# openai/blocksparse

Hardware: AMD Instinct MI355X
Metric: bsmm_effective_tflops_4096x4096_bs32_d20 (higher is better)
Workload: dtype bf16

## Files before the change

### blocksparse_amd/csrc/bsmm_common.h

```cpp
#pragma once
#include <hip/hip_runtime.h>
#include <stdint.h>

namespace bsmm {

typedef float f32x16 __attribute__((ext_vector_type(16)));
typedef float f32x4 __attribute__((ext_vector_type(4)));
typedef __bf16 bf16x8 __attribute__((ext_vector_type(8)));
typedef _Float16 f16x8 __attribute__((ext_vector_type(8)));
typedef _Float16 f16x4 __attribute__((ext_vector_type(4)));
typedef short s16x4v __attribute__((ext_vector_type(4)));

struct DTf32 {
    typedef float T;
    static constexpr bool is16 = false;
    static __device__ __forceinline__ float to_f32(float v) { return v; }
    static __device__ __forceinline__ float from_f32(float v) { return v; }
};

struct DTf16 {
    typedef uint16_t T;
    static constexpr bool is16 = true;
    static __device__ __forceinline__ float to_f32(uint16_t v) { return (float)__builtin_bit_cast(_Float16, v); }
    static __device__ __forceinline__ uint16_t from_f32(float v) {
// ... 113 lines not shown
template <class DT>
__device__ __forceinline__ void mma32(const Frag32<DT, false>& a, const Frag32<DT, false>& b, f32x16& acc) {
#pragma unroll
    for (int t = 0; t < 16; ++t) acc = __builtin_amdgcn_mfma_f32_32x32x2f32(a.v[t], b.v[t], acc, 0, 0, 0);
}

template <class DT, bool IS16 = DT::is16>
struct Frag16;

template <class DT>
struct Frag16<DT, true> {
    static constexpr int KL = 8;
    static constexpr int KS = 32;
    uint4 q;
    __device__ __forceinline__ void zero() { q = zero_u4(); }
    __device__ __forceinline__ void load_contig(const uint16_t* p) { q = *reinterpret_cast<const uint4*>(p); }
    __device__ __forceinline__ void load_contig_lim(const uint16_t* p, int lim) { q = load8_u16_lim(p, lim); }
    __device__ __forceinline__ void load_strided(const uint16_t* p, size_t stride) { q = gather8_u16(p, stride); }
    __device__ __forceinline__ void load_strided_lim(const uint16_t* p, size_t stride, int lim) { q = gather8_u16_lim(p, stride, lim); }
};

template <class DT>
struct Frag16<DT, false> {
    static constexpr int KL = 4;
    static constexpr int KS = 16;
    float v[4];
    __device__ __forceinline__ void zero() { v[0] = v[1] = v[2] = v[3] = 0.f; }
    __device__ __forceinline__ void load_contig(const float* p) {
        float4 x = *reinterpret_cast<const float4*>(p);
        v[0] = x.x; v[1] = x.y; v[2] = x.z; v[3] = x.w;
    }
    __device__ __forceinline__ void load_contig_lim(const float* p, int lim) {
        if (lim >= 4) { load_contig(p); return; }
#pragma unroll
        for (int t = 0; t < 4; ++t) v[t] = (t < lim) ? p[t] : 0.f;
    }
    __device__ __forceinline__ void load_strided(const float* p, size_t stride) {
#pragma unroll
        for (int t = 0; t < 4; ++t) v[t] = p[(size_t)t * stride];
    }
    __device__ __forceinline__ void load_strided_lim(const float* p, size_t stride, int lim) {
#pragma unroll
        for (int t = 0; t < 4; ++t) v[t] = (t < lim) ? p[(size_t)t * stride] : 0.f;
    }
};

template <class DT>
__device__ __forceinline__ void mma16(const Frag16<DT, true>& a, const Frag16<DT, true>& b, f32x4& acc) {
    acc = DT::mfma16(a.q, b.q, acc);
}
template <class DT>
__device__ __forceinline__ void mma16(const Frag16<DT, false>& a, const Frag16<DT, false>& b, f32x4& acc) {
#pragma unroll
    for (int t = 0; t < 4; ++t) acc = __builtin_amdgcn_mfma_f32_16x16x4f32(a.v[t], b.v[t], acc, 0, 0, 0);
}

template <class DT>
__device__ __forceinline__ void atomic_accumulate(typename DT::T* p, float v) {
    if constexpr (!DT::is16) {
        __hip_atomic_fetch_add(p, v, __ATOMIC_RELAXED, __HIP_MEMORY_SCOPE_AGENT);
    } else {
        uintptr_t a = reinterpret_cast<uintptr_t>(p);
        uint32_t* wp = reinterpret_cast<uint32_t*>(a & ~(uintptr_t)3);
        const bool hi = (a & 2) != 0;
        uint32_t old = __hip_atomic_load(wp, __ATOMIC_RELAXED, __HIP_MEMORY_SCOPE_AGENT);
        uint32_t assumed;
        do {
            assumed = old;
            uint16_t cur = hi ? (uint16_t)(assumed >> 16) : (uint16_t)(assumed & 0xffffu);
            uint32_t nv = DT::from_f32(DT::to_f32(cur) + v);
            uint32_t nw = hi ? ((assumed & 0x0000ffffu) | (nv << 16)) : ((assumed & 0xffff0000u) | nv);
            old = atomicCAS(wp, assumed, nw);
        } while (old != assumed);
    }
}

typedef __bf16 bf16x2_t __attribute__((ext_vector_type(2)));
typedef float f32x2_t __attribute__((ext_vector_type(2)));
__device__ __forceinline__ uint32_t bf16_pack2(float lo, float hi) {
    const f32x2_t v = {lo, hi};
    return __builtin_bit_cast(uint32_t, __builtin_convertvector(v, bf16x2_t));
}

struct PtrList8 {
    const void* p[8];
};

__device__ __forceinline__ void glds16_asm(const void* gsrc, uint32_t lds_byte_addr) {
    unsigned keep;
    asm volatile("s_mov_b32 %0, m0\n\ts_mov_b32 m0, %2\n\ts_nop 0\n\tglobal_load_lds_dwordx4 %1, off\n\ts_mov_b32 m0, %0"
                 : "=&s"(keep)
                 : "v"(gsrc), "s"(lds_byte_addr)
                 : "memory");
}
__device__ __forceinline__ void glds16_asm_masked(const void* gsrc, uint32_t lds_byte_addr, uint64_t mask) {
    unsigned keep;
    asm volatile("s_mov_b32 %0, m0\n\ts_mov_b32 m0, %2\n\ts_mov_b64 exec, %3\n\ts_nop 0\n\tglobal_load_lds_dwordx4 %1, off\n\t"
                 "s_mov_b64 exec, -1\n\ts_mov_b32 m0, %0"
                 : "=&s"(keep)
                 : "v"(gsrc), "s"(lds_byte_addr), "s"(mask)
                 : "memory");
}
__device__ __forceinline__ uint32_t lds_addr_of(const void* p) {
    return (uint32_t)(uintptr_t)(__attribute__((address_space(3))) const void*)p;
}

}
```

### blocksparse_amd/csrc/bsmm_updat_v2.h

```cpp
#pragma once
#include <type_traits>

#include "bsmm_common.h"
#include "bsmm_plan.h"
#include "bsmm_updat_tr.h"

namespace bsmm {

#ifndef U2_NT_PARTS
#define U2_NT_PARTS 1
#endif
#ifndef U2_MAX_SLICES
#define U2_MAX_SLICES 8
#endif
#ifndef U2_CH_ROWS
#define U2_CH_ROWS 16
#endif
#ifndef U2_SETB_FROM
#define U2_SETB_FROM 0
#endif
constexpr int U2_CH = U2_CH_ROWS;
constexpr int U2_KS = U2_CH / 16;
constexpr int U2_D = 64 / U2_CH;
constexpr int U2_AHEAD = U2_D / 2;
static_assert(U2_CH == 16 || U2_CH == 32, "chunk = 1 or 2 K-steps");
constexpr int u2_ring(int ws) { return ws == 32 ? 2 : U2_D; }
constexpr int u2_lds_bytes(int ws) { return u2_ring(ws) * 2 * U2_CH * ws * 64; }
constexpr int U2_CH0 = 32;
#ifndef U2_RING5
#define U2_RING5 0
#endif
constexpr int u2_lds_bytes0(int ws) { return U2_RING5 ? 5 * ws * 32 * (U2_CH0 * 2) : 131072; }

#ifdef U2_STAMPS
__device__ unsigned long long g_u2_trace[1024 * 8];
#define U2_STAMP(k, v) do { if (wave == 0 && lane == 0 && blockIdx.x < 1024) g_u2_trace[blockIdx.x * 8 + (k)] = (v); } while (0)
#else
#define U2_STAMP(k, v) do { } while (0)
#endif

__device__ __forceinline__ const void* uniform_ptr(const void* p) {
    const uint64_t v = reinterpret_cast<uint64_t>(p);
    const uint32_t lo = __builtin_amdgcn_readfirstlane((uint32_t)v), hi = __builtin_amdgcn_readfirstlane((uint32_t)(v >> 32));
    return reinterpret_cast<const void*>(((uint64_t)hi << 32) | lo);
}

__device__ __forceinline__ void glds16_saddr(const void* sbase, uint32_t voff, uint32_t lds_byte_addr) {
    unsigned keep;
    asm volatile("s_mov_b32 %0, m0\n\ts_mov_b32 m0, %3\n\ts_nop 0\n\tglobal_load_lds_dwordx4 %1, %2\n\ts_mov_b32 m0, %0"
                 : "=&s"(keep)
                 : "v"(voff), "s"(sbase), "s"(lds_byte_addr)
                 : "memory");
}
__device__ __forceinline__ void glds16_saddr_x2(const void* sbase, uint32_t voff0, uint32_t voff1, uint32_t lds_byte_addr) {
    unsigned keep;
    asm volatile("s_mov_b32 %0, m0\n\ts_mov_b32 m0, %4\n\ts_nop 0\n\tglobal_load_lds_dwordx4 %1, %3\n\t"
                 "s_add_u32 m0, m0, 0x400\n\ts_nop 0\n\tglobal_load_lds_dwordx4 %2, %3\n\ts_mov_b32 m0, %0"
                 : "=&s"(keep)
                 : "v"(voff0), "v"(voff1), "s"(sbase), "s"(lds_byte_addr)
                 : "memory", "scc");
}

__device__ __forceinline__ void glds16_saddr_x4(const void* sbase, uint32_t v0, uint32_t v1, uint32_t v2, uint32_t v3, uint32_t lds_byte_addr) {
    unsigned keep;
    asm volatile("s_mov_b32 %0, m0\n\ts_mov_b32 m0, %6\n\ts_nop 0\n\tglobal_load_lds_dwordx4 %1, %5\n\t"
                 "s_add_u32 m0, m0, 0x400\n\ts_nop 0\n\tglobal_load_lds_dwordx4 %2, %5\n\t"
                 "s_add_u32 m0, m0, 0x400\n\ts_nop 0\n\tglobal_load_lds_dwordx4 %3, %5\n\t"
                 "s_add_u32 m0, m0, 0x400\n\ts_nop 0\n\tglobal_load_lds_dwordx4 %4, %5\n\ts_mov_b32 m0, %0"
                 : "=&s"(keep)
                 : "v"(v0), "v"(v1), "v"(v2), "v"(v3), "s"(sbase), "s"(lds_byte_addr)
                 : "memory", "scc");
}

__device__ __forceinline__ const unsigned char* pick_ptr(const PtrList8& l, int idx) {
    const void* p = l.p[0];
#pragma unroll
    for (int k = 1; k < 8; ++k) p = (idx == k) ? l.p[k] : p;
    return static_cast<const unsigned char*>(p);
}

template <class DT, int LDSB>
__device__ __forceinline__ void u2_direct_block(const PtrList8& Xs, const PtrList8& Es, float* __restrict__ scratch, const int32_t* __restrict__ plan,
                                                int N, int Cf, int Kf, int pcount, int e, long region0, unsigned char* smem) {
    typedef typename DT::T T;
    constexpr int SLOT = 2048, D = LDSB / U2_WAVES / SLOT;
    static_assert(D >= 2 && LDSB >= U2_WAVES * 4096, "direct blocks: a ring of two chunks per wave and 64 KiB for the reduction");
    const int lane = threadIdx.x & 63;
    const int wave = __builtin_amdgcn_readfirstlane(threadIdx.x >> 6);
    const int DP = plan[30];
    const int d = e / DP, q = e - d * DP;
    const int32_t* de = plan + plan[29] + 4 * d;
    const int c = __builtin_amdgcn_readfirstlane(de[1]), k = __builtin_amdgcn_readfirstlane(de[2]);
    unsigned char* ring = smem + wave * (D * SLOT);
    const uint32_t ring_addr = lds_addr_of(ring);
    const int drow = lane >> 2, dpiece = lane & 3;
    const int g16 = lane >> 4, t16 = lane & 15, h = g16 >> 1;
    const int rd_base = (8 * h + (t16 >> 2)) * 64 + (16 * (g16 & 1) + 4 * (t16 & 3)) * 2;
    f32x16 acc;
#pragma unroll
    for (int i = 0; i < 16; ++i) acc[i] = 0.f;
    const int nch = (N + 15) >> 4;
    const int lo = (int)((long)nch * q / DP), hi = (int)((long)nch * (q + 1) / DP);
    const int first = lo + wave;
    const int myq = hi > first ? (hi - first + U2_WAVES - 1) / U2_WAVES : 0;
    for (int p = 0; p < pcount; ++p) {
        const T* X = reinterpret_cast<const T*>(pick_ptr(Xs, p)) + c * 32 + dpiece * 8;
        const T* E = reinterpret_cast<const T*>(pick_ptr(Es, p)) + k * 32 + dpiece * 8;
        auto issue = [&](int j, int pos) {
            const int r = min((first + U2_WAVES * j) * 16 + drow, N - 1);
            const uint32_t slot = __builtin_amdgcn_readfirstlane(ring_addr + pos * SLOT);
            glds16_asm(X + (size_t)r * Cf, slot);
            glds16_asm(E + (size_t)r * Kf, slot + 1024);
        };
#pragma unroll
        for (int j = 0; j < D - 1; ++j) issue(j, j);
        int rd_pos = 0, wr_pos = D - 1;
        for (int j = 0; j < myq; ++j) {
            issue(j + D - 1, wr_pos);
            asm volatile("s_waitcnt vmcnt(%0)" ::"n"(2 * (D - 1)) : "memory");
            const unsigned char* sp = ring + rd_pos * SLOT + rd_base;
            rd_pos = (rd_pos + 1 == D) ? 0 : rd_pos + 1;
            wr_pos = (wr_pos + 1 == D) ? 0 : wr_pos + 1;
            const uint2 a0 = ds_tr16(sp), a1 = ds_tr16(sp + 4 * 64), b0 = ds_tr16(sp + 1024), b1 = ds_tr16(sp + 1024 + 4 * 64);
            uint4 a = make_uint4(a0.x, a0.y, a1.x, a1.y);
            const uint4 b = make_uint4(b0.x, b0.y, b1.x, b1.y);
            const int nb = (first + U2_WAVES * j) * 16 + 8 * h;
            if (nb + 8 > N) {
                uint32_t* u = reinterpret_cast<uint32_t*>(&a);
#pragma unroll
                for (int i = 0; i < 4; ++i) u[i] &= ((nb + 2 * i < N) ? 0xffffu : 0u) | ((nb + 2 * i + 1 < N) ? 0xffff0000u : 0u);
            }
            asm volatile("s_waitcnt lgkmcnt(0)" ::: "memory");
            acc = DT::mfma32(a, b, acc);
        }
        asm volatile("s_waitcnt vmcnt(0)" ::: "memory");
    }
    __syncthreads();
    float* red = reinterpret_cast<float*>(smem);
#pragma unroll
    for (int reg = 0; reg < 16; ++reg) red[wave * 1024 + reg * 64 + lane] = acc[reg];
    __syncthreads();
    float sum = 0.f;
#pragma unroll
    for (int v = 0; v < U2_WAVES; ++v) sum += red[v * 1024 + threadIdx.x];
    const int reg = threadIdx.x >> 6, ln = threadIdx.x & 63;
    float* region = scratch + ((size_t)region0 * (U2_WAVES * U2_SLOTS) + (size_t)e) * 1024;
    region[((reg >> 2) * 64 + ln) * 4 + (reg & 3)] = sum;
}

template <class DT, int WS, int AXIS = 1>
__global__ void __launch_bounds__(64 * U2_WAVES, 4)
updat32_a1_v2_kernel(PtrList8 Xs, PtrList8 Es, typename DT::T* __restrict__ DW, float* __restrict__ scratch,
                     const int32_t* __restrict__ plan, int N, int Cf, int Kf, int pcount, float alpha, float beta, int flat, int main_grid, int rounds) {
    typedef typename DT::T T;
    static_assert(DT::is16 && (WS == 8 || WS == 16 || (WS == 32 && AXIS == 1)), "updat v2: 16-bit storage types, 8x8 / 16x16 windows (32x32: feature axis 1)");
    extern __shared__ __attribute__((aligned(16))) unsigned char smem[];
    constexpr int CH = AXIS == 1 ? U2_CH : U2_CH0;
    constexpr int KS = CH / 16;
    constexpr bool FIVE = AXIS == 0 && U2_RING5;
    constexpr int D = AXIS == 1 ? u2_ring(WS) : (WS == 16 ? 2 : 4);
    constexpr int AHEAD = D / 2;
    constexpr int ROWB = AXIS == 1 ? WS * 64 : CH * 2;
    constexpr int SLAB = AXIS == 1 ? CH * ROWB : WS * 32 * ROWB;
    constexpr int SLOT = 2 * SLAB;
    constexpr int PPR = ROWB / 16;
    constexpr int RPI = ROWB <= 1024 ? 1024 / ROWB : 1;
    constexpr int IPR = ROWB <= 1024 ? 1 : ROWB / 1024;
    constexpr int IPO = SLAB / 1024;
    constexpr int NI = 2 * IPO / U2_WAVES;
    static_assert((NI == 1 || NI == 2 || NI == 4) && NI * U2_WAVES == 2 * IPO && IPO % NI == 0, "the chunk must split evenly over the waves");

    const int mg = main_grid > 0 ? main_grid : (int)gridDim.x;
    if ((int)blockIdx.x >= mg) {
        if constexpr (AXIS == 1) u2_direct_block<DT, u2_lds_bytes(WS)>(Xs, Es, scratch, plan, N, Cf, Kf, pcount, (int)blockIdx.x - mg, (long)rounds * mg, smem);
        return;
    }
    const int lane = threadIdx.x & 63;
    const int wave = __builtin_amdgcn_readfirstlane(threadIdx.x >> 6);
    const int32_t* items = plan + plan[6];
    const int nchunks = (N + CH - 1) / CH;
    const int nfull = N / CH;
    const int CPI = pcount * nchunks;
    const bool xcd_mode = flat == 0 && (mg & 7) == 0;
    const int nsets = xcd_mode ? plan[8] : 1;
    const int nparts = xcd_mode ? 8 / nsets : 1;
    const int U = xcd_mode ? mg >> 3 : mg;
    const int xcd = xcd_mode ? (blockIdx.x & 7) : 0, uj = xcd_mode ? (blockIdx.x >> 3) : blockIdx.x;
    const int set = xcd / nparts, part = xcd - set * nparts;
    const int set_first = xcd_mode ? plan[9 + 2 * set] : 0, set_count = xcd_mode ? plan[10 + 2 * set] : plan[4];
    const int part_lo = (int)((long)part * CPI / nparts), part_hi = (int)((long)(part + 1) * CPI / nparts);
    const int full_rounds = set_count / U, m_last = set_count - full_rounds * U;
    const int k_last = m_last > 0 ? min(U / m_last, U2_MAX_SLICES) : 0;
    const int total_rounds = full_rounds + ((m_last > 0 && uj < m_last * k_last) ? 1 : 0);

    const uint32_t base_addr = lds_addr_of(smem);
    const int opE = (NI * wave) / IPO;
    const int ii0 = (NI * wave) % IPO;
    const int d_row0 = ROWB <= 1024 ? ii0 * RPI + lane / PPR : ii0 / IPR;
    auto row_of = [&](int q) -> int { return ROWB <= 1024 ? d_row0 + q * RPI : (ii0 + q) / IPR; };
    auto pos_of = [&](int q) -> int { return ROWB <= 1024 ? lane % PPR : ((ii0 + q) % IPR) * 64 + lane; };
    const uint32_t sub_off = ii0 * 1024;
    const uint32_t wave_off = (!FIVE ? opE * SLAB : 0) + sub_off;
    constexpr uint32_t HS = SLAB, RING0 = 5 * SLAB;
    const int F = opE ? Kf : Cf;
    const int my_piece0 = (lane % PPR) ^ ((d_row0 >> 2) & 3);
    const int g16 = lane >> 4, t16 = lane & 15;
    const int h = AXIS == 1 ? g16 >> 1 : lane >> 5;
    const int trow = t16 >> 2;
    const int tsub = (2 * (g16 & 1) + ((t16 & 3) >> 1)) * 16 + (t16 & 1) * 8;
    const int frag_row = AXIS == 1 ? (8 * h + trow) * ROWB + tsub : (lane & 31) * ROWB + ((h ^ (((lane & 31) >> 2) & 3)) << 4);
#ifdef U2_NO_PINGPONG
    const bool setb = false;
#else
    constexpr int SB = U2_SETB_FROM > 0 ? U2_SETB_FROM : ((WS == 8 && AXIS == 1) ? 4 : U2_WAVES / 2);
    const bool setb = wave >= SB;
#endif

    U2_STAMP(0, __builtin_amdgcn_s_memrealtime());
    U2_STAMP(4, (unsigned long long)total_rounds);
    for (int round = 0; round < total_rounds; ++round) {
        int item, r0, cnt;
        if (round < full_rounds) {
            item = set_first + round * U + uj;
            r0 = part_lo; cnt = part_hi - part_lo;
        } else {
            const int which = uj / k_last, slice = uj - which * k_last, L = part_hi - part_lo;
            item = set_first + full_rounds * U + which;
            r0 = part_lo + (int)((long)slice * L / k_last);
            cnt = part_lo + (int)((long)(slice + 1) * L / k_last) - r0;
        }
// ... 176 lines not shown
                    else     asm volatile("s_waitcnt vmcnt(%0)" ::"n"(NI) : "memory");
                }
                if (nfull != nchunks) {
                    if (cq == nfull) {
#pragma unroll
                        for (int e = 0; e < NI; ++e)
                            if (AXIS == 1 ? (cq * CH + row_of(e) >= N) : (cq * CH + my_piece0 * 8 >= N))
                                *reinterpret_cast<uint4*>(smem + (!FIVE ? (uint32_t)(i & (D - 1)) * SLOT : (uint32_t)((2 * i + opE) % 5) * HS) + wave_off + e * 1024 + lane * 16) = zero_u4();
                        asm volatile("s_waitcnt lgkmcnt(0)" ::: "memory");
                    }
                    if (++cq == nchunks) cq = 0;
                }
                if constexpr ((D == 2 || FIVE) && SETB) asm volatile("s_waitcnt lgkmcnt(0)" ::: "memory");
#ifndef U2_NO_BARRIER
                __builtin_amdgcn_s_barrier();
#endif
                const unsigned char* slot = smem + (!FIVE ? vslot : vslot0);
                const unsigned char* slot_y = smem + vslot;
                if constexpr (N0 == 0) {
                    U2_ISSUE();
                } else if constexpr (!SETB) {
                    read_frags(slot, slot_y, 0);
                    U2_ISSUE();
                    multiply();
#pragma unroll
                    for (int ks = 1; ks < KS; ++ks) { read_frags(slot, slot_y, ks); multiply(); }
                } else {
                    multiply();
                    __builtin_amdgcn_sched_barrier(0);
                    U2_ISSUE();
#pragma unroll
                    for (int ks = 0; ks < KS - 1; ++ks) { read_frags(slot, slot_y, ks); multiply(); }
                    read_frags(slot, slot_y, KS - 1);
                }
                if constexpr (!FIVE) {
                    vslot = (vslot + SLOT) & (D * SLOT - 1);
                } else {
                    vslot += 2 * HS;  vslot = vslot >= RING0 ? vslot - RING0 : vslot;
                    vslot0 += 2 * HS; vslot0 = vslot0 >= RING0 ? vslot0 - RING0 : vslot0;
                }
            }
#undef U2_ISSUE
#undef U2_ISSUE_SLOW
#undef U2_DMA1
#undef U2_DMA2
#undef U2_DMA4
            if constexpr (SETB && N0 > 0) multiply();
            asm volatile("s_waitcnt vmcnt(0)" ::: "memory");
            __builtin_amdgcn_s_barrier();
        };
        using std::integral_constant;
#define RUN(A, B)                                                                                                          \
    do {                                                                                                                   \
        if (setb) run(integral_constant<int, A>{}, integral_constant<int, B>{}, integral_constant<bool, true>{});          \
        else      run(integral_constant<int, A>{}, integral_constant<int, B>{}, integral_constant<bool, false>{});         \
    } while (0)
        switch (n0 * 8 + n1) {
            case 0 * 8 + 0: RUN(0, 0); break;
            case 1 * 8 + 0: RUN(1, 0); break;
            case 1 * 8 + 1: RUN(1, 1); break;
            case 1 * 8 + 2: RUN(1, 2); break;
            case 1 * 8 + 3: RUN(1, 3); break;
            case 2 * 8 + 0: RUN(2, 0); break;
            case 2 * 8 + 1: RUN(2, 1); break;
            case 2 * 8 + 2: RUN(2, 2); break;
            case 3 * 8 + 0: RUN(3, 0); break;
            case 3 * 8 + 1: RUN(3, 1); break;
            default:        RUN(4, 0); break;
        }
#undef RUN
        if (round == 0) { U2_STAMP(1, __builtin_amdgcn_s_memrealtime()); U2_STAMP(5, (unsigned long long)cnt); }

        if (scratch != nullptr) {
            float4* reg_base = reinterpret_cast<float4*>(scratch) + ((size_t)(round * mg + blockIdx.x) * (U2_WAVES * U2_SLOTS) + wave * U2_SLOTS) * 256 + lane;
#pragma unroll
            for (int j = 0; j < U2_SLOTS; ++j) {
                if (j >= n0 + n1) break;
#ifdef U2_NO_EPILOGUE
                if (alpha != 12345.f) continue;
#endif
#pragma unroll
                for (int q = 0; q < 4; ++q)
                {
#if U2_NT_PARTS
                    typedef float f4v __attribute__((ext_vector_type(4)));
                    const f4v v = {acc[j][4 * q + 0], acc[j][4 * q + 1], acc[j][4 * q + 2], acc[j][4 * q + 3]};
                    __builtin_nontemporal_store(v, reinterpret_cast<f4v*>(reg_base + (j * 4 + q) * 64));
#else
                    reg_base[(j * 4 + q) * 64] = make_float4(acc[j][4 * q + 0], acc[j][4 * q + 1], acc[j][4 * q + 2], acc[j][4 * q + 3]);
#endif
                }
            }
        } else {
#pragma unroll
            for (int j = 0; j < U2_SLOTS; ++j) {
                if (j >= n0 + n1) break;
                const int wid = __builtin_amdgcn_readfirstlane(wd[1 + j]) & 0x1fffffff;
                const size_t base = (size_t)wid * 1024 + (lane & 31);
#pragma unroll
                for (int reg = 0; reg < 16; ++reg) {
                    const int ci = (reg & 3) + 8 * (reg >> 2) + 4 * (lane >> 5);
                    const size_t idx = base + ci * 32;
#ifdef U2_NO_EPILOGUE
                    if (alpha == 12345.f) DW[idx] = DT::from_f32(acc[j][reg]);
                    continue;
#endif
                    float out = alpha * acc[j][reg];
                    if (beta != 0.f) out += beta * DT::to_f32(DW[idx]);
                    DW[idx] = DT::from_f32(out);
                }
            }
        }
        if (round == 0) U2_STAMP(2, __builtin_amdgcn_s_memrealtime());
    }
    U2_STAMP(3, __builtin_amdgcn_s_memrealtime());
}

__device__ __forceinline__ float4 u2_ld(const float4* p) {
#if U2_NT_PARTS
    typedef float f4v __attribute__((ext_vector_type(4)));
    const f4v v = __builtin_nontemporal_load(reinterpret_cast<const f4v*>(p));
    return make_float4(v.x, v.y, v.z, v.w);
#else
    return *p;
#endif
}

template <class DT, bool SUMS>
__global__ void __launch_bounds__(128)
updat2_reduce_kernel(const float* __restrict__ parts, typename DT::T* __restrict__ DW, float* __restrict__ sums, const int32_t* __restrict__ plan,
                     const int32_t* __restrict__ bmap, const float* __restrict__ gate, int direct_region0, int main_grid, int flat, int CPI, float alpha, float beta, int q64 = 0) {
    const int w = blockIdx.x;
    const int qq = threadIdx.x >> 6, l = threadIdx.x & 63;
    const int32_t bm = bmap[w];
    const bool direct = bm <= -2;
    const int item = direct ? 0 : bm >> 8, slot = direct ? 0 : bm & 255;
    const bool xcd_mode = flat == 0 && (main_grid & 7) == 0;
    const int nsets = xcd_mode ? plan[8] : 1;
    const int nparts = xcd_mode ? 8 / nsets : 1;
    const int U = xcd_mode ? main_grid >> 3 : main_grid;
    int set = 0;
    if (xcd_mode)
        for (int s = 1; s < nsets; ++s) if (item >= plan[9 + 2 * s]) set = s;
    const int set_first = xcd_mode ? plan[9 + 2 * set] : 0, set_count = xcd_mode ? plan[10 + 2 * set] : plan[4];
    const int pos = item - set_first;
    const int full_rounds = set_count / U, m_last = set_count - full_rounds * U;
    const int k_last = m_last > 0 ? min(U / m_last, U2_MAX_SLICES) : 0;
    const float4* base = reinterpret_cast<const float4*>(parts) + ((size_t)slot * 4 + qq) * 64 + l;
    constexpr size_t REGION = (size_t)U2_WAVES * U2_SLOTS * 256;
    const bool sliced = pos >= full_rounds * U;
    const int which = pos - full_rounds * U;
    const float4 zero4 = make_float4(0.f, 0.f, 0.f, 0.f);
    float4 acc0 = zero4, acc1 = zero4;
    auto part_len = [&](int part) -> int {
        const unsigned part_lo = (unsigned)part * (unsigned)CPI / (unsigned)nparts, part_hi = (unsigned)(part + 1) * (unsigned)CPI / (unsigned)nparts;
        return (int)(part_hi - part_lo);
    };
    auto add = [](float4& a, const float4& v) { a.x += v.x; a.y += v.y; a.z += v.z; a.w += v.w; };
    if (direct) {
        const int dp = plan[30];
        const float4* p0 = base + (size_t)direct_region0 * REGION + (size_t)((-2 - bm) * dp) * 256;
        float4 v0[8], v1[8];
#pragma unroll
        for (int part = 0; part < 8; ++part) {
            v0[part] = v1[part] = zero4;
            if (part < dp) { v0[part] = u2_ld(p0 + (size_t)part * 256); v1[part] = u2_ld(p0 + (size_t)part * 256 + 128); }
        }
#pragma unroll
        for (int part = 0; part < 8; ++part) { add(acc0, v0[part]); add(acc1, v1[part]); }
    } else if (!sliced) {
        const int round = pos / U, uj = pos - round * U;
        float4 v0[8], v1[8];
#pragma unroll
        for (int part = 0; part < 8; ++part) {
            v0[part] = v1[part] = zero4;
            if (part < nparts && part_len(part) > 0) {
                const int xcd = set * nparts + part;
                const float4* p = base + ((size_t)round * main_grid + (xcd_mode ? uj * 8 + xcd : uj)) * REGION;
                v0[part] = u2_ld(p); v1[part] = u2_ld(p + 128);
            }
        }
#pragma unroll
        for (int part = 0; part < 8; ++part) { add(acc0, v0[part]); add(acc1, v1[part]); }
    } else {
        for (int part = 0; part < nparts; ++part) {
            const int L = part_len(part);
            if (L <= 0) continue;
            const int xcd = set * nparts + part;
            const float4* rb = base + (size_t)full_rounds * main_grid * REGION;
            auto where = [&](int slice) -> const float4* {
                if (slice >= k_last) return nullptr;
                if (L < k_last) {
                    const unsigned lo = (unsigned)slice * (unsigned)L / (unsigned)k_last, hi = (unsigned)(slice + 1) * (unsigned)L / (unsigned)k_last;
                    if (hi == lo) return nullptr;
                }
                const int uj = which * k_last + slice;
                return rb + (size_t)(xcd_mode ? uj * 8 + xcd : uj) * REGION;
            };
            for (int sl = 0; sl < k_last; sl += 8) {
                float4 a[8], b[8];
#pragma unroll
                for (int e = 0; e < 8; ++e) {
                    const float4* p = where(sl + e);
                    a[e] = b[e] = zero4;
                    if (p) { a[e] = u2_ld(p); b[e] = u2_ld(p + 128); }
                }
#pragma unroll
                for (int e = 0; e < 8; ++e) { add(acc0, a[e]); add(acc1, b[e]); }
            }
        }
    }
#pragma unroll
    for (int hq = 0; hq < 2; ++hq) {
        const int q = qq + 2 * hq;
        const float4 acc = hq ? acc1 : acc0;
        const float r[4] = {acc.x, acc.y, acc.z, acc.w};
        const int row = 8 * q + 4 * (l >> 5), col = l & 31;
        const size_t o = q64 ? (size_t)(w >> 2) * 4096 + (size_t)(32 * ((w >> 1) & 1) + row) * 64 + 32 * (w & 1) + col : (size_t)w * 1024 + (size_t)row * 32 + col;
        const int ostep = q64 ? 64 : 32;
        if constexpr (SUMS) {
#pragma unroll
            for (int e = 0; e < 4; ++e) sums[o + e * ostep] = r[e];
        } else {
            const float a = gate ? alpha * gate[q64 ? w >> 2 : w] : alpha;
#pragma unroll
            for (int e = 0; e < 4; ++e) {
                float v = a * r[e];
                if (beta != 0.f) v += beta * DT::to_f32(DW[o + e * ostep]);
                DW[o + e * ostep] = DT::from_f32(v);
            }
        }
    }
}

template <class DT>
__global__ void __launch_bounds__(256)
updat_finalize_gated_kernel(const float* __restrict__ scratch, typename DT::T* __restrict__ DW, size_t n, int bsq, float alpha, float beta,
                            const float* __restrict__ gate, const int32_t* __restrict__ skip_if = nullptr) {
    const size_t i = ((size_t)blockIdx.x * 256 + threadIdx.x) * 4;
    if (i >= n || (skip_if && skip_if[0] != 0)) return;
    const float4 s = *reinterpret_cast<const float4*>(scratch + i);
    const float a = gate ? alpha * gate[i / bsq] : alpha;
    float v[4] = {a * s.x, a * s.y, a * s.z, a * s.w};
    if (beta != 0.f) {
#pragma unroll
        for (int e = 0; e < 4; ++e) v[e] += beta * DT::to_f32(DW[i + e]);
    }
#pragma unroll
    for (int e = 0; e < 4; ++e) DW[i + e] = DT::from_f32(v[e]);
}

}
```

### blocksparse_amd/csrc/bsmm_xflow.h

```cpp
#pragma once
#include "bsmm_common.h"
#include "bsmm_plan.h"
#include "bsmm_updat_v2.h"
#include "bsmm_updat_tr.h"
#include "bsmm_xprop.h"

namespace bsmm {

#ifndef X4_NO_XDMA
#define X4_NO_XDMA 0
#endif
#ifndef X4_NO_WDMA
#define X4_NO_WDMA 0
#endif
#ifndef X4_NO_MATH
#define X4_NO_MATH 0
#endif
#ifndef X4_READS_FIRST
#define X4_READS_FIRST 1
#endif
#ifndef X4_PUBLISH_FIRST
#define X4_PUBLISH_FIRST 1
#endif
#ifndef X4_FETCH_EARLY
#define X4_FETCH_EARLY 0
#endif
#ifndef X4_STAGGER
#define X4_STAGGER 0
#endif
#ifndef X4_PRIO
#define X4_PRIO 0
#endif
#ifdef X4_TIMELINE
__device__ unsigned long long g_x4_tl[256 * 40];
#define X4_TL(step, k) do { if (blockIdx.x == 0 && (step) < 256) { const unsigned long long t_ = __builtin_readcyclecounter(); if (lane == 0) g_x4_tl[(step) * 40 + (k)] = t_; } } while (0)
#else
#define X4_TL(step, k) do { } while (0)
#endif
#ifdef X4_STAMPS
__device__ unsigned long long g_x4_trace[64 * 16 * 8];
#define X4_T0() const unsigned long long t0_ = __builtin_readcyclecounter()
#define X4_T1(k) tacc[k] += __builtin_readcyclecounter() - t0_
#else
#define X4_T0() do { } while (0)
#define X4_T1(k) do { } while (0)
#endif
constexpr int X4_R = 128;
constexpr int X4_SLAB = X4_R * 128;
constexpr int X4_S = 2;
constexpr int X4_WBASE = X4_D * X4_SLAB;
constexpr int X4_WWAVE = X4_S * 2048;
constexpr int X4_FLAGS = X4_WBASE + X4_G * X4_WWAVE;
constexpr int X4_LDS = X4_FLAGS + 64 + 64;
constexpr int X4_DI = 16 / X4_PARTS;
static_assert(X4_LDS <= 163840, "flow kernel: ring must fit the LDS");
static_assert(X4_WWAVE >= 64 * 64, "the epilogue stages 64 rows x 64 B per pass in a wave's weight slots");
static_assert((X4_WWAVE & (X4_WWAVE - 1)) == 0 && X4_WBASE % X4_WWAVE == 0, "weight slot toggling by XOR needs aligned slots");

__device__ __forceinline__ void x4_lane_write(uint64_t em, uint32_t v_addr, uint32_t v_value) {
    asm volatile("s_mov_b64 exec, %0\n\tds_write_b32 %1, %2\n\ts_mov_b64 exec, -1" ::"s"(em), "v"(v_addr), "v"(v_value) : "memory");
}
__device__ __forceinline__ void x4_lane_add(uint64_t em, uint32_t v_addr, uint32_t v_value) {
    asm volatile("s_mov_b64 exec, %0\n\tds_add_u32 %1, %2\n\ts_mov_b64 exec, -1" ::"s"(em), "v"(v_addr), "v"(v_value) : "memory");
}
__device__ __forceinline__ void x4_lane_poll_ge(uint64_t em, uint32_t v_addr, uint32_t v_target) {
    uint32_t t;
    asm volatile("s_mov_b64 exec, %1\n"
                 "1:\n\tds_read_b32 %0, %2\n\ts_waitcnt lgkmcnt(0)\n\tv_cmp_ge_u32 vcc, %0, %3\n\ts_cbranch_vccnz 2f\n\ts_sleep 1\n\ts_branch 1b\n"
                 "2:\n\ts_mov_b64 exec, -1"
                 : "=&v"(t) : "s"(em), "v"(v_addr), "v"(v_target) : "memory", "vcc");
}
__device__ __forceinline__ void x4_poll_all_ge(uint32_t v_addr, uint32_t s_need) {
    uint32_t t;
    asm volatile("1:\n\tds_read_b32 %0, %1\n\ts_waitcnt lgkmcnt(0)\n\tv_cmp_gt_u32 vcc, %2, %0\n\ts_cbranch_vccz 2f\n\ts_sleep 1\n\ts_branch 1b\n2:"
                 : "=&v"(t) : "v"(v_addr), "s"(s_need) : "memory", "vcc");
}

#ifndef X4_XPOL
#define X4_XPOL ""
#endif
__device__ __forceinline__ void x4_glds_x(const void* sbase, uint32_t voff, uint32_t lds_byte_addr) {
    unsigned keep;
    asm volatile("s_mov_b32 %0, m0\n\ts_mov_b32 m0, %3\n\ts_nop 0\n\tglobal_load_lds_dwordx4 %1, %2" X4_XPOL "\n\ts_mov_b32 m0, %0"
                 : "=&s"(keep) : "v"(voff), "s"(sbase), "s"(lds_byte_addr) : "memory");
}
__device__ __forceinline__ void x4_glds_x4(const void* sbase, uint32_t v0, uint32_t v1, uint32_t v2, uint32_t v3, uint32_t lds_byte_addr) {
    unsigned keep;
    asm volatile("s_mov_b32 %0, m0\n\ts_mov_b32 m0, %6\n\ts_nop 0\n\tglobal_load_lds_dwordx4 %1, %5" X4_XPOL "\n\t"
                 "s_add_u32 m0, m0, 0x400\n\ts_nop 0\n\tglobal_load_lds_dwordx4 %2, %5" X4_XPOL "\n\t"
                 "s_add_u32 m0, m0, 0x400\n\ts_nop 0\n\tglobal_load_lds_dwordx4 %3, %5" X4_XPOL "\n\t"
                 "s_add_u32 m0, m0, 0x400\n\ts_nop 0\n\tglobal_load_lds_dwordx4 %4, %5" X4_XPOL "\n\ts_mov_b32 m0, %0"
                 : "=&s"(keep) : "v"(v0), "v"(v1), "v"(v2), "v"(v3), "s"(sbase), "s"(lds_byte_addr) : "memory", "scc");
}

template <int DI>
__device__ __forceinline__ void x4_wait_ctl(uint32_t ctl) {
    asm volatile("s_bitcmp1_b32 %0, 3\n\ts_cbranch_scc0 1f\n\ts_waitcnt vmcnt(2)\n\ts_branch 3f\n"
                 "1:\n\ts_bitcmp1_b32 %0, 4\n\ts_cbranch_scc0 2f\n\ts_waitcnt vmcnt(0)\n\ts_branch 3f\n"
                 "2:\n\ts_waitcnt vmcnt(%1)\n3:" ::"s"(ctl), "n"(DI) : "memory", "scc");
}

#ifdef X4_ENDSTAMPS
__device__ unsigned long long g_x4_ends[512 * 16 * 8];
#endif
template <class DT, bool TRANSW, int RT = 4>
__global__ void __launch_bounds__(64 * X4_G, 4)
xflow32_kernel(const typename DT::T* __restrict__ X, const typename DT::T* __restrict__ Wsel, typename DT::T* __restrict__ Y,
               const int32_t* __restrict__ plan, XMap map, int N, int Cin, int Kout) {
    typedef typename DT::T T;
    static_assert(DT::is16, "flow kernel: 16-bit storage types");
    static_assert(RT == 4 || RT == 2, "flow kernel: units of 128 or 64 rows");
    constexpr int R = 32 * RT, SLAB = R * 128, D = X4_D * 4 / RT, DI = X4_DI * RT / 4;
    static_assert(D * SLAB == X4_WBASE && DI % 4 == 0 && D <= 16, "flow kernel: ring geometry");
    extern __shared__ __attribute__((aligned(16))) unsigned char smem[];
    const int lane = threadIdx.x & 63;
    const int wave = __builtin_amdgcn_readfirstlane(threadIdx.x >> 6);
    const int r = lane & 31, h = lane >> 5;
    const uint32_t base_addr = lds_addr_of(smem);
    const uint32_t prog_addr = base_addr + X4_FLAGS, full_addr = base_addr + X4_FLAGS + 64;
    if (threadIdx.x < 32) reinterpret_cast<uint32_t*>(smem + X4_FLAGS)[threadIdx.x] = 0u;
    __syncthreads();
#if X4_STAGGER
    for (int i = ((blockIdx.x >> 3) & 31) * X4_STAGGER; i > 0; --i) __builtin_amdgcn_s_sleep(1);
#endif

    const int npairs_full = Cin / 64;
    const unsigned char* xt = reinterpret_cast<const unsigned char*>(X);
    const unsigned char* wsel = static_cast<const unsigned char*>(uniform_ptr(Wsel));
    const uint32_t wvoff = TRANSW ? (uint32_t)lane * 16u : (uint32_t)((lane >> 2) * 64 + (((lane & 3) ^ ((lane >> 4) & 3)) << 4));
    const uint32_t wslot0 = X4_WBASE + wave * X4_WWAVE;
    const int xsw = (r >> 1) & 7;
    uint32_t xrd[2], wrd[2];
#pragma unroll
    for (int kk = 0; kk < 2; ++kk) {
        xrd[kk] = r * 128 + (((2 * kk + h) ^ xsw) << 4);
        if constexpr (TRANSW) {
            const int g16 = lane >> 4, t16 = lane & 15;
            wrd[kk] = wslot0 + (16 * kk + 8 * h + (t16 >> 2)) * 64 + (16 * (g16 & 1) + 4 * (t16 & 3)) * 2;
        } else {
            wrd[kk] = wslot0 + r * 64 + (((2 * kk + h) ^ ((r >> 2) & 3)) << 4);
        }
    }
    const uint32_t my_prog_s = prog_addr + 4 * wave;
    const uint32_t stride16 = (uint32_t)Cin * 16u;
    const uint32_t pc_e = (uint32_t)((lane & 7) ^ (lane >> 4));
    const uint32_t vo_e = (uint32_t)(lane >> 3) * (uint32_t)Cin * 2u + pc_e * 16u;

#ifdef X4_STAMPS
    unsigned long long tacc[8] = {0, 0, 0, 0, 0, 0, 0, 0};
    const unsigned long long tstart = __builtin_readcyclecounter();
#endif
#ifdef X4_ENDSTAMPS
    int x4e_u = 0;
    if (lane == 0 && blockIdx.x < 512) g_x4_ends[(blockIdx.x * 16 + wave) * 8] = __builtin_amdgcn_s_memrealtime();
#endif
    uint32_t gs = 0;
    const int nunits = map.grid();
    for (int unit = blockIdx.x; unit < nunits; unit += gridDim.x) {
        int tile, grp;
        if (!xmap_decode(map, unit, tile, grp)) continue;
        const int32_t* gh = plan + plan[5] + X4_GROUP * grp;
        const int step_off = __builtin_amdgcn_readfirstlane(gh[0]), nsteps = __builtin_amdgcn_readfirstlane(gh[1]);
        const int list_off = __builtin_amdgcn_readfirstlane(gh[4]), lcap = __builtin_amdgcn_readfirstlane(gh[5]);
        const int32_t* pairs = plan + plan[6] + step_off;
        const int32_t* lists = plan + plan[7] + list_off;
        const int nev = __builtin_amdgcn_readfirstlane(lists[wave]);
        const int my_ob = __builtin_amdgcn_readfirstlane(lists[X4_G + wave]);
        const int32_t* mine = lists + 2 * X4_G + (size_t)2 * lcap * wave;
        const int n_tile = tile * R;
        const unsigned char* xtile = static_cast<const unsigned char*>(uniform_ptr(xt + (size_t)n_tile * Cin * 2));
        const bool fast_tile = n_tile + R <= N;

        f32x16 acc[RT];
#pragma unroll
        for (int t = 0; t < RT; ++t)
#pragma unroll
            for (int i = 0; i < 16; ++i) acc[t][i] = 0.f;
// ... 96 lines not shown
#endif
                } else if (ty_s == 2) {
                    const uint32_t g1 = (uint32_t)__builtin_amdgcn_readlane(v_g, idx);
                    { X4_T0(); if (g1 > (uint32_t)D) x4_poll_all_ge(prog_addr + 4 * (lane & 15), g1 - (uint32_t)D); X4_T1(3); }
                    X4_T0();
#ifdef X4_TIMELINE
                    const uint32_t dbg_r = (uint32_t)__builtin_amdgcn_readlane(v_dbg, idx);
                    X4_TL(dbg_r & 0xffff, dbg_r >> 16);
#endif
                    if (!X4_NO_XDMA) {
                        const uint32_t dst = base_addr + (uint32_t)__builtin_amdgcn_readlane(v_x, idx);
                        const uint32_t poff = (uint32_t)__builtin_amdgcn_readlane(v_fa, idx);
                        const uint32_t part_i = (uint32_t)__builtin_amdgcn_readlane(v_x, idx) % (uint32_t)SLAB / 1024u;
                        if (!(ctl & 128u)) {
                            const uint32_t k0 = part_i * stride16 + poff;
                            const uint32_t vo_o = (pc_e & 4u) ? vo_e - 64u : vo_e + 64u;
#pragma unroll
                            for (int k = 0; k < DI; k += 4)
                                x4_glds_x4(xtile, vo_e + (k0 + (k + 0) * stride16), vo_o + (k0 + (k + 1) * stride16), vo_e + (k0 + (k + 2) * stride16),
                                                vo_o + (k0 + (k + 3) * stride16), dst + k * 1024);
                        } else {
                            const bool tail = (int)(poff >> 7) >= npairs_full;
#pragma unroll
                            for (int k = 0; k < DI; ++k) {
                                const int row = 8 * ((int)part_i + k) + (lane >> 3);
                                const int xr = min(n_tile + row, N - 1) - n_tile;
                                const int piece = (lane & 7) ^ ((row >> 1) & 7);
                                uint32_t voff = (uint32_t)xr * (uint32_t)Cin * 2u + piece * 16 + poff;
                                if (tail && (piece & 4)) voff -= 64;
                                x4_glds_x(xtile, voff, dst + k * 1024);
                            }
                        }
                    }
                    X4_T1(4);
#ifdef X4_TIMELINE
                    X4_TL(dbg_r & 0xffff, 2 + (dbg_r >> 16));
#endif
                } else if (ty_s == 3) {
                    x4_lane_add(em, v_fa, 1u);
#ifdef X4_TIMELINE
                    { const uint32_t dbg_a = (uint32_t)__builtin_amdgcn_readlane(v_dbg, idx); X4_TL(dbg_a & 0xffff, 4 + (dbg_a >> 16)); }
#endif
                }
                if (ty_s < 2) {
                    X4_T0();
                    if (X4_PUBLISH_FIRST) x4_lane_write(em, my_prog_s, v_pv);
                    if ((ctl & 64u) && !fetched) {
                        if (!X4_NO_WDMA) {
                            const uint32_t fo = (uint32_t)__builtin_amdgcn_readlane(v_fw, idx);
                            glds16_saddr_x2(wsel, wvoff + fo, wvoff + fo + 1024u, base_addr + (wslot0 ^ s_wf));
                        }
                        s_wf ^= 2048u;
                    }
                    if (!X4_PUBLISH_FIRST) x4_lane_write(em, my_prog_s, v_pv);
                    if (X4_PRIO) __builtin_amdgcn_s_setprio(0);
                    X4_T1(5);
                }
            }
        }
        gs += (uint32_t)nsteps;

        if (my_ob >= 0) {
            unsigned char* stage = smem + wslot0;
            unsigned char* ybase = reinterpret_cast<unsigned char*>(Y + (size_t)my_ob * 32);
#pragma unroll
            for (int pass = 0; pass < RT / 2; ++pass) {
#pragma unroll
                for (int tt = 0; tt < 2; ++tt) {
                    const int t = 2 * pass + tt;
                    const int n = tt * 32 + r;
#pragma unroll
                    for (int q = 0; q < 4; ++q) {
                        const uint32_t lo = (uint32_t)DT::from_f32(acc[t][4 * q + 0]) | ((uint32_t)DT::from_f32(acc[t][4 * q + 1]) << 16);
                        const uint32_t hi = (uint32_t)DT::from_f32(acc[t][4 * q + 2]) | ((uint32_t)DT::from_f32(acc[t][4 * q + 3]) << 16);
                        *reinterpret_cast<uint2*>(stage + n * 64 + ((q ^ ((n >> 2) & 3)) << 4) + 8 * h) = make_uint2(lo, hi);
                    }
                }
                asm volatile("" ::: "memory");
#pragma unroll
                for (int i = 0; i < 4; ++i) {
                    const int n = 16 * i + (lane >> 2), pc = lane & 3;
                    const uint4 v = *reinterpret_cast<const uint4*>(stage + n * 64 + ((pc ^ ((n >> 2) & 3)) << 4));
                    const int gn = n_tile + 64 * pass + n;
                    if (gn < N) *reinterpret_cast<uint4*>(ybase + (size_t)gn * Kout * 2 + pc * 16) = v;
                }
                asm volatile("" ::: "memory");
            }
        }
#ifdef X4_ENDSTAMPS
        if (lane == 0 && blockIdx.x < 512 && x4e_u < 6) g_x4_ends[(blockIdx.x * 16 + wave) * 8 + 1 + x4e_u] = __builtin_amdgcn_s_memrealtime();
        ++x4e_u;
#endif
    }
#ifdef X4_ENDSTAMPS
    if (lane == 0 && blockIdx.x < 512) g_x4_ends[(blockIdx.x * 16 + wave) * 8 + 7] = (unsigned long long)x4e_u;
#endif
#ifdef X4_STAMPS
    tacc[6] = __builtin_readcyclecounter() - tstart;
    if (blockIdx.x < 64 && lane == 0)
        for (int k = 0; k < 8; ++k) g_x4_trace[(blockIdx.x * 16 + wave) * 8 + k] = tacc[k];
#endif
}

}
```

Baseline: 654.4.

## Stage dW epilogue tiles through LDS for vectorized 16-byte stores with cache policies

The weight-gradient epilogues now transpose accumulator fragments through shared memory, so each thread writes a contiguous 16-byte chunk of bf16 or f32 output instead of scattered 2-byte or 4-byte stores. The partial-sum reduction path is also staged through LDS and written as float4. A templated store16 helper adds selectable cache policies (plain, nt, sc1, sc0 sc1) for the partial, dW, epilogue and Y stores. The aim is to cut store-instruction count and uncoalesced writes, at the cost of extra LDS traffic, added __syncthreads, and a new static shared tile that could reduce occupancy.

```diff
diff --git a/blocksparse_amd/csrc/bsmm_common.h b/blocksparse_amd/csrc/bsmm_common.h
--- a/blocksparse_amd/csrc/bsmm_common.h
+++ b/blocksparse_amd/csrc/bsmm_common.h
@@ -219,6 +219,25 @@
     return __builtin_bit_cast(uint32_t, __builtin_convertvector(v, bf16x2_t));
 }
 
+#define ST_PLAIN 0
+#define ST_NT 1
+#define ST_SC1 2
+#define ST_SC0_SC1 3
+template <int POL>
+__device__ __forceinline__ void store16(void* p, uint4 v) {
+    static_assert(POL >= ST_PLAIN && POL <= ST_SC0_SC1, "store16: plain, nt, sc1 or sc0 sc1");
+    typedef uint32_t u32x4 __attribute__((ext_vector_type(4)));
+    const u32x4 d = {v.x, v.y, v.z, v.w};
+    if constexpr (POL == ST_PLAIN) *reinterpret_cast<uint4*>(p) = v;
+    else if constexpr (POL == ST_NT) asm volatile("global_store_dwordx4 %0, %1, off nt\n\ts_nop 1" ::"v"(p), "v"(d) : "memory");
+    else if constexpr (POL == ST_SC1) asm volatile("global_store_dwordx4 %0, %1, off sc1\n\ts_nop 1" ::"v"(p), "v"(d) : "memory");
+    else asm volatile("global_store_dwordx4 %0, %1, off sc0 sc1\n\ts_nop 1" ::"v"(p), "v"(d) : "memory");
+}
+template <int POL>
+__device__ __forceinline__ void store16(void* p, float4 v) {
+    store16<POL>(p, make_uint4(__float_as_uint(v.x), __float_as_uint(v.y), __float_as_uint(v.z), __float_as_uint(v.w)));
+}
+
 struct PtrList8 {
     const void* p[8];
 };
diff --git a/blocksparse_amd/csrc/bsmm_dw_pieces.h b/blocksparse_amd/csrc/bsmm_dw_pieces.h
--- /dev/null
+++ b/blocksparse_amd/csrc/bsmm_dw_pieces.h
@@ -0,0 +1,28 @@
+#pragma once
+#include <stddef.h>
+
+#if defined(__HIPCC__)
+#define BSMM_DWP_FN __host__ __device__ inline
+#else
+#define BSMM_DWP_FN inline
+#endif
+
+namespace bsmm {
+
+BSMM_DWP_FN int dw_acc_row(int q, int l, int e) { return 8 * q + 4 * (l >> 5) + e; }
+BSMM_DWP_FN int dw_acc_col(int l) { return l & 31; }
+BSMM_DWP_FN int dw_tile_index(int row, int col) { return row * 32 + col; }
+
+BSMM_DWP_FN int dw_piece_count(int epp) { return 1024 / epp; }
+BSMM_DWP_FN int dw_piece_row(int p, int epp) { return p / (32 / epp); }
+BSMM_DWP_FN int dw_piece_col(int p, int epp) { return (p % (32 / epp)) * epp; }
+
+BSMM_DWP_FN size_t dw_elem_offset(int w, int row, int col, int q64) {
+    return q64 ? (size_t)(w >> 2) * 4096 + (size_t)(32 * ((w >> 1) & 1) + row) * 64 + 32 * (w & 1) + col
+               : (size_t)w * 1024 + (size_t)row * 32 + col;
+}
+
+BSMM_DWP_FN int dw_thread_piece(int tid, int i, int threads) { return tid + threads * i; }
+BSMM_DWP_FN int dw_pieces_per_thread(int epp, int threads) { return dw_piece_count(epp) / threads; }
+
+}
diff --git a/blocksparse_amd/csrc/bsmm_updat_v2.h b/blocksparse_amd/csrc/bsmm_updat_v2.h
--- a/blocksparse_amd/csrc/bsmm_updat_v2.h
+++ b/blocksparse_amd/csrc/bsmm_updat_v2.h
@@ -2,6 +2,7 @@
 #include <type_traits>
 
 #include "bsmm_common.h"
+#include "bsmm_dw_pieces.h"
 #include "bsmm_plan.h"
 #include "bsmm_updat_tr.h"
 
@@ -9,6 +10,15 @@
 
 #ifndef U2_NT_PARTS
 #define U2_NT_PARTS 1
+#endif
+#ifndef U2_PPOL
+#define U2_PPOL (U2_NT_PARTS ? ST_NT : ST_PLAIN)
+#endif
+#ifndef U2_DWPOL
+#define U2_DWPOL ST_PLAIN
+#endif
+#ifndef U2_EPOL
+#define U2_EPOL ST_PLAIN
 #endif
 #ifndef U2_MAX_SLICES
 #define U2_MAX_SLICES 8
@@ -143,9 +153,15 @@
     float sum = 0.f;
 #pragma unroll
     for (int v = 0; v < U2_WAVES; ++v) sum += red[v * 1024 + threadIdx.x];
-    const int reg = threadIdx.x >> 6, ln = threadIdx.x & 63;
-    float* region = scratch + ((size_t)region0 * (U2_WAVES * U2_SLOTS) + (size_t)e) * 1024;
-    region[((reg >> 2) * 64 + ln) * 4 + (reg & 3)] = sum;
+    __syncthreads();
+    red[threadIdx.x] = sum;
+    __syncthreads();
+    if (threadIdx.x < 256) {
+        const int q = threadIdx.x >> 6, ln = threadIdx.x & 63;
+        const float4 v = make_float4(red[(4 * q + 0) * 64 + ln], red[(4 * q + 1) * 64 + ln], red[(4 * q + 2) * 64 + ln], red[(4 * q + 3) * 64 + ln]);
+        float4* region = reinterpret_cast<float4*>(scratch + ((size_t)region0 * (U2_WAVES * U2_SLOTS) + (size_t)e) * 1024);
+        store16<U2_PPOL>(region + q * 64 + ln, v);
+    }
 }
 
 template <class DT, int WS, int AXIS = 1>
@@ -488,34 +504,48 @@
 #pragma unroll
                 for (int q = 0; q < 4; ++q)
                 {
-#if U2_NT_PARTS
-                    typedef float f4v __attribute__((ext_vector_type(4)));
-                    const f4v v = {acc[j][4 * q + 0], acc[j][4 * q + 1], acc[j][4 * q + 2], acc[j][4 * q + 3]};
-                    __builtin_nontemporal_store(v, reinterpret_cast<f4v*>(reg_base + (j * 4 + q) * 64));
-#else
-                    reg_base[(j * 4 + q) * 64] = make_float4(acc[j][4 * q + 0], acc[j][4 * q + 1], acc[j][4 * q + 2], acc[j][4 * q + 3]);
-#endif
+                    store16<U2_PPOL>(reg_base + (j * 4 + q) * 64, make_float4(acc[j][4 * q + 0], acc[j][4 * q + 1], acc[j][4 * q + 2], acc[j][4 * q + 3]));
                 }
             }
         } else {
+            float* stg = reinterpret_cast<float*>(smem) + wave * 1024;
 #pragma unroll
             for (int j = 0; j < U2_SLOTS; ++j) {
                 if (j >= n0 + n1) break;
                 const int wid = __builtin_amdgcn_readfirstlane(wd[1 + j]) & 0x1fffffff;
-                const size_t base = (size_t)wid * 1024 + (lane & 31);
-#pragma unroll
-                for (int reg = 0; reg < 16; ++reg) {
-                    const int ci = (reg & 3) + 8 * (reg >> 2) + 4 * (lane >> 5);
-                    const size_t idx = base + ci * 32;
+#pragma unroll
+                for (int reg = 0; reg < 16; ++reg) stg[dw_tile_index(dw_acc_row(reg >> 2, lane, reg & 3), dw_acc_col(lane))] = acc[j][reg];
+                asm volatile("" ::: "memory");
+#pragma unroll 1
+                for (int i = 0; i < 2; ++i) {
+                    const int p = dw_thread_piece(lane, i, 64), row = dw_piece_row(p, 8), col0 = dw_piece_col(p, 8);
+                    const float4 s0 = *reinterpret_cast<const float4*>(stg + dw_tile_index(row, col0)), s1 = *reinterpret_cast<const float4*>(stg + dw_tile_index(row, col0 + 4));
+                    const float sv[8] = {s0.x, s0.y, s0.z, s0.w, s1.x, s1.y, s1.z, s1.w};
+                    T* dst = DW + dw_elem_offset(wid, row, col0, 0);
 #ifdef U2_NO_EPILOGUE
-                    if (alpha == 12345.f) DW[idx] = DT::from_f32(acc[j][reg]);
+                    if (alpha == 12345.f) store16<U2_EPOL>(dst, s0);
                     continue;
 #endif
-                    float out = alpha * acc[j][reg];
-                    if (beta != 0.f) out += beta * DT::to_f32(DW[idx]);
-                    DW[idx] = DT::from_f32(out);
-                }
-            }
+                    uint32_t ow[4] = {0u, 0u, 0u, 0u};
+                    if (beta != 0.f) {
+                        const uint4 o4 = *reinterpret_cast<const uint4*>(dst);
+                        ow[0] = o4.x; ow[1] = o4.y; ow[2] = o4.z; ow[3] = o4.w;
+                    }
+                    uint32_t pk[4];
+#pragma unroll
+                    for (int k = 0; k < 4; ++k) {
+                        float lo = alpha * sv[2 * k], hi = alpha * sv[2 * k + 1];
+                        if (beta != 0.f) {
+                            lo += beta * DT::to_f32((T)(ow[k] & 0xffffu));
+                            hi += beta * DT::to_f32((T)(ow[k] >> 16));
+                        }
+                        pk[k] = (uint32_t)DT::from_f32(lo) | ((uint32_t)DT::from_f32(hi) << 16);
+                    }
+                    store16<U2_EPOL>(dst, make_uint4(pk[0], pk[1], pk[2], pk[3]));
+                }
+                asm volatile("" ::: "memory");
+            }
+            __syncthreads();
         }
         if (round == 0) U2_STAMP(2, __builtin_amdgcn_s_memrealtime());
     }
@@ -616,26 +646,45 @@
             }
         }
     }
+    __shared__ __attribute__((aligned(16))) float tile[1024];
 #pragma unroll
     for (int hq = 0; hq < 2; ++hq) {
         const int q = qq + 2 * hq;
         const float4 acc = hq ? acc1 : acc0;
         const float r[4] = {acc.x, acc.y, acc.z, acc.w};
-        const int row = 8 * q + 4 * (l >> 5), col = l & 31;
-        const size_t o = q64 ? (size_t)(w >> 2) * 4096 + (size_t)(32 * ((w >> 1) & 1) + row) * 64 + 32 * (w & 1) + col : (size_t)w * 1024 + (size_t)row * 32 + col;
-        const int ostep = q64 ? 64 : 32;
-        if constexpr (SUMS) {
-#pragma unroll
-            for (int e = 0; e < 4; ++e) sums[o + e * ostep] = r[e];
-        } else {
-            const float a = gate ? alpha * gate[q64 ? w >> 2 : w] : alpha;
-#pragma unroll
-            for (int e = 0; e < 4; ++e) {
-                float v = a * r[e];
-                if (beta != 0.f) v += beta * DT::to_f32(DW[o + e * ostep]);
-                DW[o + e * ostep] = DT::from_f32(v);
-            }
-        }
+#pragma unroll
+        for (int e = 0; e < 4; ++e) tile[dw_tile_index(dw_acc_row(q, l, e), dw_acc_col(l))] = r[e];
+    }
+    __syncthreads();
+    if constexpr (SUMS) {
+#pragma unroll
+        for (int i = 0; i < 2; ++i) {
+            const int p = dw_thread_piece(threadIdx.x, i, 128), row = dw_piece_row(p, 4), col0 = dw_piece_col(p, 4);
+            store16<U2_DWPOL>(sums + dw_elem_offset(w, row, col0, q64), *reinterpret_cast<const float4*>(tile + dw_tile_index(row, col0)));
+        }
+    } else {
+        typedef typename DT::T T;
+        const int p = dw_thread_piece(threadIdx.x, 0, 128), row = dw_piece_row(p, 8), col0 = dw_piece_col(p, 8);
+        const float4 s0 = *reinterpret_cast<const float4*>(tile + dw_tile_index(row, col0)), s1 = *reinterpret_cast<const float4*>(tile + dw_tile_index(row, col0 + 4));
+        const float sv[8] = {s0.x, s0.y, s0.z, s0.w, s1.x, s1.y, s1.z, s1.w};
+        const float a = gate ? alpha * gate[q64 ? w >> 2 : w] : alpha;
+        T* dst = DW + dw_elem_offset(w, row, col0, q64);
+        uint32_t ow[4] = {0u, 0u, 0u, 0u};
+        if (beta != 0.f) {
+            const uint4 o4 = *reinterpret_cast<const uint4*>(dst);
+            ow[0] = o4.x; ow[1] = o4.y; ow[2] = o4.z; ow[3] = o4.w;
+        }
+        uint32_t pk[4];
+#pragma unroll
+        for (int k = 0; k < 4; ++k) {
+            float lo = a * sv[2 * k], hi = a * sv[2 * k + 1];
+            if (beta != 0.f) {
+                lo += beta * DT::to_f32((T)(ow[k] & 0xffffu));
+                hi += beta * DT::to_f32((T)(ow[k] >> 16));
+            }
+            pk[k] = (uint32_t)DT::from_f32(lo) | ((uint32_t)DT::from_f32(hi) << 16);
+        }
+        store16<U2_DWPOL>(dst, make_uint4(pk[0], pk[1], pk[2], pk[3]));
     }
 }
 
diff --git a/blocksparse_amd/csrc/bsmm_xflow.h b/blocksparse_amd/csrc/bsmm_xflow.h
--- a/blocksparse_amd/csrc/bsmm_xflow.h
+++ b/blocksparse_amd/csrc/bsmm_xflow.h
@@ -93,6 +93,9 @@
                  : "=&s"(keep) : "v"(v0), "v"(v1), "v"(v2), "v"(v3), "s"(sbase), "s"(lds_byte_addr) : "memory", "scc");
 }
 
+#ifndef X4_YPOL
+#define X4_YPOL ST_PLAIN
+#endif
 template <int DI>
 __device__ __forceinline__ void x4_wait_ctl(uint32_t ctl) {
     asm volatile("s_bitcmp1_b32 %0, 3\n\ts_cbranch_scc0 1f\n\ts_waitcnt vmcnt(2)\n\ts_branch 3f\n"
@@ -355,7 +358,7 @@
                     const int n = 16 * i + (lane >> 2), pc = lane & 3;
                     const uint4 v = *reinterpret_cast<const uint4*>(stage + n * 64 + ((pc ^ ((n >> 2) & 3)) << 4));
                     const int gn = n_tile + 64 * pass + n;
-                    if (gn < N) *reinterpret_cast<uint4*>(ybase + (size_t)gn * Kout * 2 + pc * 16) = v;
+                    if (gn < N) store16<X4_YPOL>(ybase + (size_t)gn * Kout * 2 + pc * 16, v);
                 }
                 asm volatile("" ::: "memory");
             }
```

Result: no change. 652.7 (-0.3%).
